# coezbek/Zonos

Hardware: AMD Instinct MI355X
Metric: DAC codes/sec (end-to-end generate + DAC decode), Zonos-v0.1-transformer batch=64/GPU (higher is better)
Workload: dtype bf16; 1 GPU; c3: B=64/GPU, Lc=400, prefix 10, 2580 new tokens (30 s), EOS disabled, CLI sampling (linear .65 conf .4 rep 2.5/8), DAC decode of all codes; model=Zonos-v0.1-transformer, global_batch=64, seq_len=2999, parallelism=dp1

## Files before the change

include/zonos_hip.h:

```cpp
#ifndef ZONOS_HIP_H
#define ZONOS_HIP_H
#include <stddef.h>
#include <stdint.h>

#ifdef __cplusplus
extern "C" {
#endif

int zk_version(void);
const char* zk_last_error(void);
int zk_device_sync(void);
long zk_abi_size(int which);

typedef struct zk_sampling_params {
    float temperature;
    float top_p;
    float min_p;
    float linear, conf, quad;
    int32_t top_k;
    int32_t rp_window;
    float cfg_scale;
    int32_t force_full_length;
} zk_sampling_params;

// ... 271 lines not shown
int zk_dac_rvq_decode(const int64_t* codes, int B, int ncb, int T, long code_bstride,
                      const float* tables, int ncode, int hidden, float* z, int Tz,
                      const int32_t* lens, void* stream);
int zk_dac_conv(const float* in, int B, int Cin, int Tin, const float* alpha,
                const float* w, const float* bias, int Cout, int ks, int dil, int pad,
                int Qn, int out_stride, int out_off, float* out, int Tout, const float* resid,
                int do_tanh, const int32_t* lens, int in_scale, int out_scale, void* stream);
int zk_dac_prep_convt(const float* w, int Cin, int Cout, int s, float* w_out, void* stream);

int zk_dac_prep_w16(const float* w, int Cout, int Cin, int ks, int s, int mode, uint16_t* w_hi,
                    uint16_t* w_lo, void* stream);
int zk_dac_conv16(const float* in, int B, int Cin, int Tin, const float* alpha, const uint16_t* w_hi,
                  const uint16_t* w_lo, const float* bias, int Cout, int ks, int dil, int pad,
                  int Qn, int out_stride, int out_off, float* out, int Tout, const float* resid,
                  int do_tanh, const int32_t* lens, int in_scale, int out_scale, int npass, void* stream);
int zk_dac_tail(const float* in, int B, int C, int T, const float* alpha, const float* w,
                const float* bias, float* out, const int32_t* lens, int scale, void* stream);

int zk_dac_rvq_decode_cl(const int64_t* codes, int B, int ncb, int T, long code_bstride,
                         const float* tables, int ncode, int hidden, int cpad, uint16_t* z,
                         const int32_t* lens, void* stream);
int zk_dac_conv_cl(const uint16_t* in, int B, int Cin, int Tin, const uint16_t* w, long w_phase_stride,
                   const float* bias, int Cout, int ks, int dil, int pad, int Qn, int nphase,
                   int out_stride, int out_off0, int Tout, const float* resid, float* x_out,
                   const float* alpha_next, void* s_out, int s_f32, const int32_t* lens, int in_scale,
                   int out_scale, void* stream);
int zk_dac_resunit_supported(int C);
int zk_dac_resunit_cl(const uint16_t* s_in, int B, int C, int T, const uint16_t* w7, const float* b7, int dil,
                      const float* a2, const uint16_t* w1, const float* b1, float* x, const float* alpha_next,
                      void* s_out, int s_f32, const int32_t* lens, int scale, void* stream);
#define ZK_DAC_PLAN_N 9
int zk_dac_conv_plan(int fused, int B, int Cin, int Cout, int ks, int dil, int Qn, int nphase, int resid,
                     int s_f32, int32_t* plan);
int zk_dac_tail_cl(const float* s, int B, int C, int T, const float* w, const float* bias,
                   float* out, const int32_t* lens, int scale, void* stream);

#define ZK_DAC_MAXB 6
#define ZK_DAC_MAXR 3
typedef struct zk_dac_resunit {
    int32_t dil;
    const float* a1;
    const uint16_t* w1;
    const float* b1;
    const float* a2;
    const uint16_t* w2;
    const float* b2;
} zk_dac_resunit;
typedef struct zk_dac_block {
    int32_t stride, cin, cout, nres;
    const float* alpha;
    const uint16_t* wt;
    const float* bt;
    zk_dac_resunit res[ZK_DAC_MAXR];
} zk_dac_block;
typedef struct zk_dac_desc {
    int32_t nblocks, ncb, codebook_size, hidden, cin0, c0;
    const float* tables;
    const uint16_t* conv1_w;
    const float* conv1_b;
    const float* final_alpha;
    const float* conv2_w;
    const float* conv2_b;
    zk_dac_block blocks[ZK_DAC_MAXB];
} zk_dac_desc;
size_t zk_dac_decode_workspace(const zk_dac_desc* d, int B, int T);
int zk_dac_decode(const zk_dac_desc* d, const int64_t* codes, int B, int T, const int32_t* lens, void* workspace,
// ... 107 lines not shown
```

zonos_amd/_lib.py:

```python
from __future__ import annotations

import ctypes as C
import os

import torch

_HERE = os.path.dirname(os.path.abspath(__file__))
LIB_PATH = os.environ.get("ZK_LIB_PATH") or os.path.join(_HERE, "lib", "libzonos_hip.so")

P = C.c_void_p
I = C.c_int
L = C.c_long
F = C.c_float
U64 = C.c_uint64
I64 = C.c_int64


class SamplingParams(C.Structure):
    _fields_ = [("temperature", F), ("top_p", F), ("min_p", F), ("linear", F), ("conf", F), ("quad", F),
                ("top_k", C.c_int32), ("rp_window", C.c_int32), ("cfg_scale", F),
                ("force_full_length", C.c_int32)]


class GenState(C.Structure):
# ... 167 lines not shown
}

_lib = None


class ZonosHipError(RuntimeError):
    pass


def load():
    global _lib
    if _lib is not None:
        return _lib
    if not os.path.exists(LIB_PATH):
        raise ZonosHipError(f"{LIB_PATH} not found: build it with `python -m zonos_amd.build` "
                            "(there is no CPU fallback)")
    lib = C.CDLL(LIB_PATH)
    for name, args in _SIGS.items():
        fn = getattr(lib, name)
        fn.argtypes = args
        fn.restype = C.c_int
    lib.zk_last_error.restype = C.c_char_p
    lib.zk_last_error.argtypes = []
    lib.zk_loudness_max_blocks.restype = C.c_int
    lib.zk_loudness_max_blocks.argtypes = [L, I]
    lib.zk_abi_size.restype = C.c_long
    lib.zk_abi_size.argtypes = [I]
    lib.zk_dac_decode_workspace.restype = C.c_size_t
    lib.zk_dac_decode_workspace.argtypes = [C.POINTER(DacDesc), I, I]
    lib.zk_stream_workspace.restype = C.c_size_t
    lib.zk_stream_workspace.argtypes = [C.POINTER(StreamDesc), I]
    lib.zk_dac_resunit_supported.restype = C.c_int
    lib.zk_dac_resunit_supported.argtypes = [I]
    lib.zk_gemm_warm_tiles.restype = C.c_int
    lib.zk_gemm_warm_tiles.argtypes = [I, I, I, I, I, I]
    lib.zk_torch_noise_policy.restype = C.c_int
    lib.zk_torch_noise_policy.argtypes = [L, I, I, C.POINTER(C.c_int), C.POINTER(C.c_long)]
    lib.zk_spk_conv_tiles.restype = C.c_int
    lib.zk_spk_conv_tiles.argtypes = [I, I]
    lib.zk_speaker_workspace_bytes.restype = C.c_size_t
    lib.zk_speaker_workspace_bytes.argtypes = [C.POINTER(SpkDesc), I, I]
    _lib = lib
    return lib


def exported_symbols() -> list[str]:
    return list(_SIGS) + ["zk_last_error", "zk_loudness_max_blocks", "zk_abi_size",
                          "zk_dac_decode_workspace", "zk_stream_workspace", "zk_dac_resunit_supported", "zk_gemm_warm_tiles",
                          "zk_torch_noise_policy", "zk_spk_conv_tiles", "zk_speaker_workspace_bytes"]


def call(name: str, *args):
    lib = load()
    if len(args) != len(_SIGS[name]):
        raise TypeError(f"{name}: {len(args)} arguments given, the C ABI takes {len(_SIGS[name])}")
    rc = getattr(lib, name)(*args)
    if rc != 0:
        raise ZonosHipError(f"{name} failed ({rc}): {lib.zk_last_error().decode()}")
    return rc


DAC_PLAN_FIELDS = ("shape", "fm", "tile", "dx", "nx", "lds", "nq", "tiles", "wg_per_cu")


def dac_conv_plan(B, Cin, Cout, ks, dil, Qn, nphase=1, resid=False, s_f32=False, fused=False) -> dict:
    plan = (C.c_int32 * len(DAC_PLAN_FIELDS))()
    call("zk_dac_conv_plan", int(fused), B, Cin, Cout, ks, dil, Qn, nphase, int(resid), int(s_f32), plan)
    return dict(zip(DAC_PLAN_FIELDS, plan))


def ptr(t) -> int | None:
    if t is None:
        return None
    return t.data_ptr()


def stream_ptr(device=None) -> int:
    return torch.cuda.current_stream(device).cuda_stream


def device_index(device) -> int:
    device = torch.device(device)
    return device.index if device.index is not None else torch.cuda.current_device()


def require_gpu(t: torch.Tensor, name: str = "tensor"):
    if not t.is_cuda:
        raise ZonosHipError(f"{name} must be a GPU tensor (the HIP engine has no CPU path)")
```

zonos_amd/csrc/dac_cl.hip:

```cpp
#include "common.h"
#include "../../include/zonos_hip.h"
#include <algorithm>
#include <stdlib.h>

namespace {

typedef __attribute__((ext_vector_type(8))) _Float16 f16x8;
typedef __attribute__((ext_vector_type(4))) float f32x4;

constexpr int MAXSPAN = 64;

__device__ __attribute__((aligned(256))) uint4 g_zero_page[16];

template <int CI>
struct Img {
    static constexpr int G = CI / 8;
    static constexpr int RB = CI * 2;
    static constexpr int RPB = 256 / RB;
    static constexpr int RPR = 4096 / RB;
    ZK_DEV static int swz(int row) { return (int)(((unsigned)row / RPB) % G); }
    ZK_DEV static int off(int row, int g) { return row * RB + ((g ^ swz(row)) << 4); }
};

ZK_DEV f16x8 as_h8(uint4 v) { return __builtin_bit_cast(f16x8, v); }
// ... 17 lines not shown

ZK_DEV void wait_vm(int n) {
#define ZK_W1(N_) case N_: asm volatile("s_waitcnt vmcnt(" #N_ ")" ::: "memory"); break;
#define ZK_W8(B_) ZK_W1(B_ + 0) ZK_W1(B_ + 1) ZK_W1(B_ + 2) ZK_W1(B_ + 3) ZK_W1(B_ + 4) ZK_W1(B_ + 5) ZK_W1(B_ + 6) ZK_W1(B_ + 7)
    switch (n < 0 ? 0 : (n > 63 ? 63 : n)) {
        ZK_W8(0) ZK_W8(8) ZK_W8(16) ZK_W8(24) ZK_W8(32) ZK_W8(40) ZK_W8(48) ZK_W8(56)
        default: asm volatile("s_waitcnt vmcnt(0)" ::: "memory"); break;
    }
#undef ZK_W8
#undef ZK_W1
}

#ifndef ZK_CL_DA
#define ZK_CL_DA 3
#endif
#ifdef ZK_CL_PROF
__device__ uint64_t g_clprof[64][3][64];
__device__ uint64_t g_clprof_end[64][2];
__device__ uint64_t g_clprof_rt[64][6];
__device__ uint64_t g_clwg[4096][2];
__device__ uint32_t g_clhw[4096][8];
#define ZK_CL_STAMP(role, st)                                                                          \
    do {                                                                                               \
        if (blockIdx.x < 64 && (st) < 64 && lane == 0) g_clprof[blockIdx.x][role][st] = __builtin_amdgcn_s_memtime(); \
    } while (0)
#else
#define ZK_CL_STAMP(role, st) do { } while (0)
#endif
constexpr int CL_DA = ZK_CL_DA;
#ifndef ZK_CL_NLD
#define ZK_CL_NLD 2
#endif
constexpr int CL_NLD = ZK_CL_NLD;

constexpr int RU_XPD = 4;
template <int NQ_, int DA_, int OCC_, int NWY_, int NLDK_, int NWM_, bool FUSE_, int FMF_ = 0>
struct ConvShape {
    static constexpr int NQ = NQ_, DA = DA_, OCC = OCC_, NWY = NWY_, NLDK = NLDK_, NWM = NWM_, FMF = FMF_;
    static constexpr bool FUSE = FUSE_;
    static constexpr int THREADS = 64 * (NWM * NWY + NLDK);
    static constexpr int QTT = 16 * NQ * NWY;
    static constexpr int co_t(int fm) { return 16 * fm * NWM; }
    static constexpr bool w1lds(int fm) { return FUSE && OCC == 1 && co_t(fm) * (co_t(fm) + 8) * 2 <= 24 * 1024; }
};
using ShapePair = ConvShape<4, CL_DA, 2, 2, CL_NLD, 2, false>;
using ShapeFat = ConvShape<8, CL_DA, 1, 4, 4, 2, false>;
using ShapeFused96 = ConvShape<4, CL_DA, 1, 8, 4, 1, true, 6>;
using ShapeFused192 = ConvShape<2, CL_DA, 1, 8, 4, 1, true, 12>;

struct ConvLds {
    int ws, nws, ept, w1;
    static constexpr int pieces(int win) { return (win + 15) >> 4; }
    static constexpr int xs(int nxp) { return nxp * 1024; }
    template <class P> constexpr P xring(P base) const { return base + nws * ws; }
    template <class P> constexpr P tables(P base, int nx, int xs_) const { return xring(base) + nx * xs_; }
    template <class P> constexpr P w1img(P base, int nx, int xs_) const { return tables(base, nx, xs_) + 2 * ept; }
    constexpr int bytes(int nx, int xs_) const { return w1img(0, nx, xs_) + w1; }
};
template <class S>
constexpr ConvLds conv_lds(int fm) {
    const int co_t = S::co_t(fm);
    return ConvLds{co_t * 64, S::DA + 2, (S::FUSE ? 6 : 3) * co_t * (int)sizeof(float),
                   S::w1lds(fm) ? co_t * (co_t + 8) * 2 : 0};
}

template <class S, int FM, bool SF32, bool RES>
__global__ __launch_bounds__(S::THREADS, (S::OCC * S::THREADS + 255) / 256) void k_conv_cl(
    const uint16_t* __restrict__ in, int Cin, int Tin, const uint16_t* __restrict__ w, long wphase,
    const float* __restrict__ bias, int Cout, int ks, int dil, int pad, int Qn, int nphase, int out_stride,
    int out_off0, int Tout, const float* resid, float* xout, const float* __restrict__ alpha,
    void* __restrict__ sout, int s_f32, const int32_t* __restrict__ lens, int in_scale, int out_scale, int nq,
    int nx_slots, int dx, int B, const uint16_t* __restrict__ w1x1, const float* __restrict__ b1x1,
    const float* __restrict__ alpha_out) {
    constexpr int NQ = S::NQ, DA = S::DA, NWY = S::NWY, NLDK = S::NLDK, NWM = S::NWM;
    constexpr bool FUSE = S::FUSE;
    constexpr ConvLds LDS = conv_lds<S>(FM);
// ... 2 lines not shown
    constexpr int CO_T = S::co_t(FM);
    constexpr int WS = LDS.ws;
    static_assert(WS == CO_T * I::RB, "weight slot = CO_T image rows");
    constexpr int NWP = CO_T / 16;
    constexpr int NCW = NWM * NWY;
    static_assert(!FUSE || (NWM == 1 && !RES), "fused residual unit: one channel wave, residual in the epilogue");
    constexpr int W1S = CO_T + 8;
    constexpr bool W1LDS = S::w1lds(FM);
    constexpr int QTT = S::QTT;
    extern __shared__ __attribute__((aligned(16))) char smem[];

    const int nco = (Cout / CO_T) * nphase;
    const int ntiles = B * nq * nco;
    const int kx = blockIdx.x >> 3, nper = gridDim.x >> 3;
    const int lo = (int)((long)(blockIdx.x & 7) * ntiles / 8), hi = (int)((long)((blockIdx.x & 7) + 1) * ntiles / 8);
    const int nt = hi - lo > kx ? (hi - lo - kx + nper - 1) / nper : 0;
    auto tile_of = [&](int i, int& b, int& phase, int& co0, int& q0) {
        const int L = lo + kx + i * nper;
        const int cot = L % nco;
        b = L / (nco * nq);
        q0 = ((L / nco) % nq) * QTT;
        phase = cot % nphase;
        co0 = (cot / nphase) * CO_T;
    };

    const int tid = threadIdx.x, lane = tid & 63, wv = __builtin_amdgcn_readfirstlane(tid >> 6);
    const int win = QTT + (ks - 1) * dil;
    const int nxp = ConvLds::pieces(win);
    const int XS = ConvLds::xs(nxp);
    constexpr int NWS = LDS.nws;
    char* const wring = smem;
    char* const xring = LDS.xring(smem);
    const int nchunk = Cin / CI, nstep = nchunk * ks;

#ifdef ZK_CL_PROF
    if (blockIdx.x < 4096 && lane == 0 && wv < 6) {
        g_clhw[blockIdx.x][wv] = __builtin_amdgcn_s_getreg((31 << 11) | 4);
        if (wv == 0) g_clhw[blockIdx.x][6] = __builtin_amdgcn_s_getreg((31 << 11) | 20);
    }
    if (wv == 0 && blockIdx.x < 4096 && lane == 0) g_clwg[blockIdx.x][0] = __builtin_amdgcn_s_memrealtime();
    if (wv == 0 && blockIdx.x < 64 && lane == 0) {
        g_clprof_rt[blockIdx.x][0] = __builtin_amdgcn_s_memrealtime();
        g_clprof_rt[blockIdx.x][4] = __builtin_amdgcn_s_memtime();
    }
#endif
    if (wv >= NCW) {
        const int lw = __builtin_amdgcn_readfirstlane(wv - NCW);
        const size_t wtap = (size_t)Cout * Cin;
        static_assert((16 / I::RPB) % I::G == 0, "piece-invariant swizzle needs 16-row pieces to span whole swizzle periods");
        const int prow = lane >> 2, pslot = lane & 3;
        const int g = pslot ^ I::swz(prow);
        const int loff = prow * Cin + g * 8;
        const long prs = 16L * Cin;
        const int nxl = (nxp - lw + NLDK - 1) / NLDK, nwl = (NWP - lw + NLDK - 1) / NLDK;
        int ix = 0, tx = 0, cx = 0, u0 = 0, len_in = Tin;
        bool xfast = false;
        const uint16_t* xsrc0 = in;
        auto set_xtile = [&](int i) {
            int b_, ph_, co_, q_;
            tile_of(i, b_, ph_, co_, q_);
            len_in = lens ? min(lens[b_] * in_scale, Tin) : Tin;
            u0 = q_ - pad;
            xsrc0 = in + (size_t)b_ * Tin * Cin + loff + (long)u0 * Cin;
            xfast = u0 >= 0 && u0 + nxp * 16 <= len_in;
        };
        int iw = 0, tw = 0, cw = 0;
        const uint16_t* wsrc0 = w;
        auto set_wtile = [&](int i) {
            int b_, ph_, co_, q_;
            tile_of(i, b_, ph_, co_, q_);
            wsrc0 = w + (size_t)ph_ * wphase + (size_t)co_ * Cin + loff;
        };
        if (nt > 0) {
            set_xtile(0);
            set_wtile(0);
        }
        int xslot = 0, wslot = 0;
        int hist[DA + 1] = {};
        const int total = nt * nstep;
        for (int j = -dx; j < total; ++j) {
            int nl = 0;
            if (ix < nt) {
                if (tx == 0) {
                    char* dst = xring + xslot * XS;
                    const uint16_t* src = xsrc0 + cx * CI;
                    if (xfast) {
                        for (int p = lw; p < nxp; p += NLDK)
                            __builtin_amdgcn_global_load_lds((const void*)(src + p * prs), (void*)(dst + p * 1024), 16,
                                                             0, 0);
                    } else {
                        for (int p = lw; p < nxp; p += NLDK) {
                            const int row = p * 16 + prow, u = u0 + row;
                            const void* sp = (row < win && u >= 0 && u < len_in) ? (const void*)(src + p * prs)
                                                                                 : (const void*)g_zero_page;
                            __builtin_amdgcn_global_load_lds(sp, (void*)(dst + p * 1024), 16, 0, 0);
                        }
                    }
                    nl += nxl;
                    if (++xslot == nx_slots) xslot = 0;
                }
                if (++tx == ks) {
                    tx = 0;
                    if (++cx == nchunk) {
                        cx = 0;
                        if (++ix < nt) set_xtile(ix);
                    }
                }
            }
            if (j + DA >= 0 && iw < nt) {
                char* dst = wring + wslot * WS;
                const uint16_t* src = wsrc0 + tw * wtap + cw * CI;
#pragma unroll
                for (int pp = 0; pp < (NWP + NLDK - 1) / NLDK; ++pp) {
                    const int p = pp * NLDK + lw;
                    if (p >= NWP) break;
                    __builtin_amdgcn_global_load_lds((const void*)(src + p * prs), (void*)(dst + p * 1024), 16, 0, 0);
                }
                nl += nwl;
                if (++wslot == NWS) wslot = 0;
                if (++tw == ks) {
                    tw = 0;
                    if (++cw == nchunk) {
                        cw = 0;
                        if (++iw < nt) set_wtile(iw);
                    }
                }
            }
#pragma unroll
            for (int k = 0; k < DA; ++k) hist[k] = hist[k + 1];
            hist[DA] = nl;
            if (j >= 0) {
                int pend = 0;
#pragma unroll
                for (int k = 1; k <= DA; ++k) pend += hist[k];
                if (lw == 0) ZK_CL_STAMP(0, j);
                wait_vm(pend);
                __builtin_amdgcn_s_barrier();
                if (lw == 0) ZK_CL_STAMP(1, j);
            }
        }
        return;
    }

    const int ln = lane & 15, lg = lane >> 4, wm = wv / NWY, wn = wv % NWY;
    int t = 0, xslot = 0, wslot = 0;
    constexpr int NE = FUSE ? 6 : 3;
    static_assert(LDS.ept == NE * CO_T * (int)sizeof(float), "epilogue table = NE rows of CO_T floats");
    uint16_t* const w1img = reinterpret_cast<uint16_t*>(LDS.w1img(smem, nx_slots, XS));
    if constexpr (W1LDS) {
        for (int i = tid; i < CO_T * CO_T / 8; i += 64 * NCW) {
            const int row = i / (CO_T / 8), c8 = i % (CO_T / 8);
            *reinterpret_cast<uint4*>(w1img + row * W1S + c8 * 8) =
                *reinterpret_cast<const uint4*>(w1x1 + (size_t)row * CO_T + c8 * 8);
        }
    }
    for (int it = 0; it < nt; ++it) {
        int b, phase, co0, q0;
        tile_of(it, b, phase, co0, q0);
        f32x4 acc[FM][NQ];
#pragma unroll
        for (int m = 0; m < FM; ++m)
#pragma unroll
            for (int n = 0; n < NQ; ++n) acc[m][n] = f32x4{0.f, 0.f, 0.f, 0.f};

        float* const ept = reinterpret_cast<float*>(LDS.tables(smem, nx_slots, XS)) + (it & 1) * NE * CO_T;
        for (int i = tid; i < CO_T; i += 64 * NCW) {
            const float a_ = (FUSE || sout) ? alpha[co0 + i] : 1.f;
            ept[i] = bias[co0 + i];
            ept[CO_T + i] = a_;
            ept[2 * CO_T + i] = __fdiv_rn(1.0f, __fadd_rn(a_, 1e-9f));
            if constexpr (FUSE) {
                const float an = alpha_out[i];
                ept[3 * CO_T + i] = b1x1[i];
                ept[4 * CO_T + i] = an;
                ept[5 * CO_T + i] = __fdiv_rn(1.0f, __fadd_rn(an, 1e-9f));
            }
        }
        asm volatile("s_waitcnt lgkmcnt(0)" ::: "memory");
        const int len_out = lens ? lens[b] * out_scale : Tout;

        float4 rv[RES ? FM : 1][NQ];
        if constexpr (RES) {
#pragma unroll
            for (int m = 0; m < FM; ++m)
#pragma unroll
                for (int n = 0; n < NQ; ++n) {
                    const int q = q0 + wn * 16 * NQ + n * 16 + ln;
                    const int tt = min(max(q * out_stride + out_off0 + phase, 0), Tout - 1);
                    rv[m][n] = *reinterpret_cast<const float4*>(
                        resid + ((size_t)b * Tout + tt) * Cout + co0 + wm * 16 * FM + m * 16 + lg * 4);
                }
        }

        for (int s = 0; s < nstep; ++s) {
            __builtin_amdgcn_s_barrier();
            asm volatile("" ::: "memory");
            if (wv == 0 && it == 0) ZK_CL_STAMP(2, s);
#ifdef ZK_CL_PROF
            if (it == 0 && s == 0 && wv == 0 && blockIdx.x < 64 && lane == 0)
                g_clprof_rt[blockIdx.x][1] = __builtin_amdgcn_s_memrealtime();
#endif
            const char* xb = xring + xslot * XS;
            const char* wb = wring + wslot * WS;
            if (++wslot == NWS) wslot = 0;
            uint4 a[FM], bq[NQ];
#pragma unroll
            for (int m = 0; m < FM; ++m)
                a[m] = *reinterpret_cast<const uint4*>(wb + I::off(wm * 16 * FM + m * 16 + ln, lg));
#pragma unroll
            for (int n = 0; n < NQ; ++n)
                bq[n] = *reinterpret_cast<const uint4*>(xb + I::off(wn * 16 * NQ + n * 16 + ln + t * dil, lg));
#pragma unroll
            for (int m = 0; m < FM; ++m)
#pragma unroll
                for (int n = 0; n < NQ; ++n)
                    acc[m][n] = __builtin_amdgcn_mfma_f32_16x16x32_f16(as_h8(a[m]), as_h8(bq[n]), acc[m][n], 0, 0, 0);
            if (++t == ks) {
                t = 0;
                if (++xslot == nx_slots) xslot = 0;
            }
        }

#ifdef ZK_CL_PROF
        if (it == 0 && wv == 0 && blockIdx.x < 64 && lane == 0) {
            float keep = 0.f;
#pragma unroll
            for (int m = 0; m < FM; ++m)
#pragma unroll
                for (int n = 0; n < NQ; ++n) keep += acc[m][n][0];
            g_clprof_end[blockIdx.x][0] = __builtin_amdgcn_s_memtime() + (keep == 1.2345f);
            g_clprof_rt[blockIdx.x][2] = __builtin_amdgcn_s_memrealtime();
        }
#endif
        const int out_off = out_off0 + phase;
        if constexpr (FUSE) {
            uint2 h[FM][NQ];
#pragma unroll
            for (int m = 0; m < FM; ++m) {
                const int cl = m * 16 + lg * 4;
                const float4 bb = *reinterpret_cast<const float4*>(ept + cl);
                const float4 aa = *reinterpret_cast<const float4*>(ept + CO_T + cl);
                const float4 rr = *reinterpret_cast<const float4*>(ept + 2 * CO_T + cl);
#pragma unroll
                for (int n = 0; n < NQ; ++n)
                    h[m][n] = pack_h4(snake_fast(__fadd_rn(acc[m][n][0], bb.x), aa.x, rr.x),
                                      snake_fast(__fadd_rn(acc[m][n][1], bb.y), aa.y, rr.y),
                                      snake_fast(__fadd_rn(acc[m][n][2], bb.z), aa.z, rr.z),
                                      snake_fast(__fadd_rn(acc[m][n][3], bb.w), aa.w, rr.w));
            }
            constexpr int XPD = RU_XPD < FM ? RU_XPD : FM;
            float4 xr[XPD][NQ];
            auto load_x = [&](int mo, int buf) {
#pragma unroll
                for (int n = 0; n < NQ; ++n) {
                    const int q = q0 + wn * 16 * NQ + n * 16 + ln;
                    const int tt = min(max(q * out_stride + out_off, 0), Tout - 1);
                    xr[buf][n] = *reinterpret_cast<const float4*>(resid + ((size_t)b * Tout + tt) * Cout + mo * 16 + lg * 4);
                }
            };
#pragma unroll
            for (int p = 0; p < XPD; ++p) load_x(p, p);
            const uint16_t* w1p = w1x1;
            asm volatile("" : "+s"(w1p));
            uint2 wf[2][W1LDS ? 1 : FM];
            auto load_w = [&](int mo, int buf) {
                if constexpr (!W1LDS) {
// ... 16 lines not shown
#pragma unroll
                    for (int n = 0; n < NQ; ++n)
                        z[n] = __builtin_amdgcn_mfma_f32_16x16x16f16(as_h4(wa), as_h4(h[m][n]), z[n], 0, 0, 0);
                }
                const int co = mo * 16 + lg * 4;
                const float4 bb = *reinterpret_cast<const float4*>(ept + 3 * CO_T + co);
                const float4 aa = *reinterpret_cast<const float4*>(ept + 4 * CO_T + co);
                const float4 rr = *reinterpret_cast<const float4*>(ept + 5 * CO_T + co);
#pragma unroll
                for (int n = 0; n < NQ; ++n) {
                    const int q = q0 + wn * 16 * NQ + n * 16 + ln;
                    const int tt = q * out_stride + out_off;
                    if (q >= Qn || tt < 0 || tt >= Tout) continue;
                    const size_t o = ((size_t)b * Tout + tt) * Cout + co;
                    float v0 = 0.f, v1 = 0.f, v2 = 0.f, v3 = 0.f;
                    if (tt < len_out) {
                        const float4 r = xr[mo % XPD][n];
                        v0 = __fadd_rn(r.x, __fadd_rn(z[n][0], bb.x));
                        v1 = __fadd_rn(r.y, __fadd_rn(z[n][1], bb.y));
                        v2 = __fadd_rn(r.z, __fadd_rn(z[n][2], bb.z));
                        v3 = __fadd_rn(r.w, __fadd_rn(z[n][3], bb.w));
                    }
                    *reinterpret_cast<float4*>(xout + o) = make_float4(v0, v1, v2, v3);
                    if (SF32)
                        reinterpret_cast<float4*>(sout)[o >> 2] =
                            make_float4(snake(v0, aa.x), snake(v1, aa.y), snake(v2, aa.z), snake(v3, aa.w));
                    else
                        *reinterpret_cast<uint2*>(reinterpret_cast<uint16_t*>(sout) + o) =
                            pack_h4(snake_fast(v0, aa.x, rr.x), snake_fast(v1, aa.y, rr.y),
                                    snake_fast(v2, aa.z, rr.z), snake_fast(v3, aa.w, rr.w));
                }
                if (mo + XPD < FM) load_x(mo + XPD, mo % XPD);
            }
            continue;
        }
#pragma unroll
        for (int m = 0; m < FM; ++m) {
            const int cl = wm * 16 * FM + m * 16 + lg * 4, co = co0 + cl;
            const float4 bb = *reinterpret_cast<const float4*>(ept + cl);
            const float4 aa = *reinterpret_cast<const float4*>(ept + CO_T + cl);
            const float4 rr = *reinterpret_cast<const float4*>(ept + 2 * CO_T + cl);
            const float r0 = rr.x, r1 = rr.y, r2 = rr.z, r3 = rr.w;
#pragma unroll
            for (int n = 0; n < NQ; ++n) {
                const int q = q0 + wn * 16 * NQ + n * 16 + ln;
                const int tt = q * out_stride + out_off;
                if (q >= Qn || tt < 0 || tt >= Tout) continue;
                const size_t o = ((size_t)b * Tout + tt) * Cout + co;
                float v0 = 0.f, v1 = 0.f, v2 = 0.f, v3 = 0.f;
                if (tt < len_out) {
                    v0 = __fadd_rn(acc[m][n][0], bb.x);
                    v1 = __fadd_rn(acc[m][n][1], bb.y);
                    v2 = __fadd_rn(acc[m][n][2], bb.z);
                    v3 = __fadd_rn(acc[m][n][3], bb.w);
                    if constexpr (RES) {
                        const float4 r = rv[m][n];
                        v0 = __fadd_rn(r.x, v0);
                        v1 = __fadd_rn(r.y, v1);
                        v2 = __fadd_rn(r.z, v2);
                        v3 = __fadd_rn(r.w, v3);
                    }
                }
                if (xout) *reinterpret_cast<float4*>(xout + o) = make_float4(v0, v1, v2, v3);
                if (!sout) continue;
                if (SF32)
                    reinterpret_cast<float4*>(sout)[o >> 2] =
                        make_float4(snake(v0, aa.x), snake(v1, aa.y), snake(v2, aa.z), snake(v3, aa.w));
                else
                    *reinterpret_cast<uint2*>(reinterpret_cast<uint16_t*>(sout) + o) =
                        pack_h4(snake_fast(v0, aa.x, r0), snake_fast(v1, aa.y, r1), snake_fast(v2, aa.z, r2),
                                snake_fast(v3, aa.w, r3));
            }
        }
#ifdef ZK_CL_PROF
        if (it == 0 && wv == 0 && blockIdx.x < 64 && lane == 0) {
            asm volatile("s_waitcnt vmcnt(0)" ::: "memory");
            g_clprof_rt[blockIdx.x][3] = __builtin_amdgcn_s_memrealtime();
            g_clprof_rt[blockIdx.x][5] = __builtin_amdgcn_s_memtime();
        }
#endif
    }
#ifdef ZK_CL_PROF
    if (wv == 0 && blockIdx.x < 4096 && lane == 0) {
        asm volatile("s_waitcnt vmcnt(0)" ::: "memory");
        g_clwg[blockIdx.x][1] = __builtin_amdgcn_s_memrealtime();
    }
#endif
}

__global__ __launch_bounds__(256) void k_rvq_cl(const int64_t* __restrict__ codes, int ncb, int T, long bstr,
                                                const float* __restrict__ tables, int ncode, int hidden, int cpad,
                                                uint16_t* __restrict__ z, const int32_t* __restrict__ lens) {
    const int t = blockIdx.x, b = blockIdx.y;
    const int len = lens ? lens[b] : T;
    for (int ch = threadIdx.x * 4; ch < cpad; ch += 1024) {
        float s[4] = {0.f, 0.f, 0.f, 0.f};
        if (t < len && ch < hidden) {
            for (int k = 0; k < ncb; ++k) {
                int64_t cd = codes[b * bstr + (size_t)k * T + t];
                cd = cd < 0 ? 0 : (cd >= ncode ? ncode - 1 : cd);
                const float4 e = *reinterpret_cast<const float4*>(tables + ((size_t)k * ncode + cd) * hidden + ch);
                if (k == 0) {
                    s[0] = e.x; s[1] = e.y; s[2] = e.z; s[3] = e.w;
                } else {
                    s[0] = __fadd_rn(s[0], e.x); s[1] = __fadd_rn(s[1], e.y);
                    s[2] = __fadd_rn(s[2], e.z); s[3] = __fadd_rn(s[3], e.w);
                }
            }
        }
        *reinterpret_cast<uint2*>(z + ((size_t)b * T + t) * cpad + ch) = pack_h4(s[0], s[1], s[2], s[3]);
    }
}

constexpr int TAIL_T = 128;
// ... 167 lines not shown
template <class F>
auto with_shape(int shape, F&& f) {
    return shape == SHAPE_FAT ? f(ShapeFat{}) : shape == SHAPE_FUSED96 ? f(ShapeFused96{})
         : shape == SHAPE_FUSED192 ? f(ShapeFused192{}) : f(ShapePair{});
}
struct ConvPlan { int shape, fm, qt, dx, nx, lds, nq, tiles, occ; };

int conv_plan(const char* name, bool fused, int B, int Cin, int Cout, int ks, int dil, int Qn, int nphase, bool resid,
              bool s_f32, ConvPlan& p) {
    if (fused) {
        ZK_REQUIRE(Cout == 96 || Cout == 192, "%s: C=%d (the fused unit is built for C = 96 and 192)", name, Cout);
        ZK_REQUIRE(dil >= 1 && 6 * dil <= MAXSPAN, "%s: dil=%d", name, dil);
        ks = 7, nphase = 1;
        p.shape = Cout == 96 ? SHAPE_FUSED96 : SHAPE_FUSED192, p.fm = Cout / 16;
    } else {
        ZK_REQUIRE(Cin > 0 && Cin % 32 == 0, "%s: Cin=%d must be a multiple of 32", name, Cin);
        ZK_REQUIRE(Cout > 0 && Cout % 32 == 0, "%s: Cout=%d must be a multiple of 32", name, Cout);
        ZK_REQUIRE(ks >= 1 && ks <= 7 && dil >= 1 && (ks - 1) * dil <= MAXSPAN, "%s: ks=%d dil=%d", name, ks, dil);
        ZK_REQUIRE(nphase >= 1, "%s: bad arguments", name);
        const int nco = Cout / 32;
        p.fm = nco % 4 == 0 ? 4 : (nco % 3 == 0 ? 3 : (nco % 2 == 0 ? 2 : 1));
        p.shape = (!resid && !s_f32 && nphase == 1 && p.fm <= 3) ? SHAPE_FAT : SHAPE_PAIR;
    }
    return with_shape(p.shape, [&](auto shape) -> int {
        using S = decltype(shape);
        const ConvLds lay = conv_lds<S>(p.fm);
        const int xs = ConvLds::xs(ConvLds::pieces(S::QTT + (ks - 1) * dil));
        const int cap = 160 * 1024 / S::OCC;
        for (p.dx = std::max(S::DA, ks);; --p.dx) {
            p.nx = 1 + (p.dx + ks) / ks, p.lds = lay.bytes(p.nx, xs);
            if (p.dx <= S::DA || p.lds <= cap) break;
        }
        ZK_REQUIRE(p.lds <= 160 * 1024, "%s: LDS %d too large (Cout %d ks %d dil %d)", name, p.lds, Cout, ks, dil);
        p.qt = S::QTT, p.occ = S::OCC;
        p.nq = Qn > 0 ? (Qn + S::QTT - 1) / S::QTT : 0;
        const long tiles = (long)B * p.nq * (Cout / S::co_t(p.fm)) * nphase;
        ZK_REQUIRE(tiles < (1L << 31), "%s: too many tiles", name);
        p.tiles = (int)tiles;
        return 0;
    });
}

template <class S>
constexpr bool conv_has(int fm, bool sf32, bool res) {
    return S::FUSE ? (fm == S::FMF && !res) : S::OCC == 1 ? (fm <= 3 && !sf32 && !res) : fm <= 4;
}

template <class K, class... A>
int conv_launch_kernel(K kern, int threads, const ConvPlan& p, const char* name, hipStream_t st, A... args) {
    const size_t lds = (size_t)p.lds;
    const void* fn = reinterpret_cast<const void*>(kern);
    if (lds > 65536) (void)hipFuncSetAttribute(fn, hipFuncAttributeMaxDynamicSharedMemorySize, (int)lds);
    int dev = 0, ncu = 0, occ = 0;
    ZK_HIP(hipGetDevice(&dev));
    ZK_HIP(hipDeviceGetAttribute(&ncu, hipDeviceAttributeMultiprocessorCount, dev));
    ZK_HIP(hipOccupancyMaxActiveBlocksPerMultiprocessor(&occ, fn, threads, lds));
    ZK_REQUIRE(occ >= 1, "%s: kernel does not fit a CU (LDS %zu)", name, lds);
    const long resident = (long)ncu * occ / 8 * 8;
    const long grid = std::min<long>(((long)p.tiles + 7) / 8 * 8, std::max<long>(resident, 8));
    hipLaunchKernelGGL(kern, dim3((unsigned)grid), dim3(threads), lds, st, args...);
    ZK_CHECK_LAUNCH(name);
    return 0;
}

template <class... A>
int conv_launch(const ConvPlan& p, bool sf32, bool res, const char* name, hipStream_t st, A... args) {
// ... 47 lines not shown
    hipLaunchKernelGGL(k_rvq_cl, dim3(T, B), dim3(256), 0, (hipStream_t)stream, codes, ncb, T, code_bstride, tables,
                       ncode, hidden, cpad, z, lens);
    ZK_CHECK_LAUNCH("zk_dac_rvq_decode_cl");
    return 0;
}

extern "C" int zk_dac_conv_cl(const uint16_t* in, int B, int Cin, int Tin, const uint16_t* w, long w_phase_stride,
                              const float* bias, int Cout, int ks, int dil, int pad, int Qn, int nphase,
                              int out_stride, int out_off0, int Tout, const float* resid, float* x_out,
                              const float* alpha_next, void* s_out, int s_f32, const int32_t* lens, int in_scale,
                              int out_scale, void* stream) {
    const char* const name = "zk_dac_conv_cl";
    ConvPlan p;
    ZK_TRY(conv_plan(name, false, B, Cin, Cout, ks, dil, Qn, nphase, resid != nullptr, s_f32 != 0, p));
    ZK_REQUIRE(bias != nullptr && (s_out == nullptr || alpha_next != nullptr) && (s_out != nullptr || x_out != nullptr),
               "zk_dac_conv_cl: bad arguments");
    if (B == 0 || Qn <= 0) return 0;
    return conv_launch(p, s_f32 != 0, resid != nullptr, name, (hipStream_t)stream, in, Cin, Tin, w, w_phase_stride, bias,
                       Cout, ks, dil, pad, Qn, nphase, out_stride, out_off0, Tout, resid, x_out, alpha_next, s_out, s_f32,
                       lens, in_scale, out_scale, p.nq, p.nx, p.dx, B, nullptr, nullptr, nullptr);
}

extern "C" int zk_dac_conv_plan(int fused, int B, int Cin, int Cout, int ks, int dil, int Qn, int nphase, int resid,
                                int s_f32, int32_t* plan) {
    ConvPlan p;
    ZK_REQUIRE(plan != nullptr, "zk_dac_conv_plan: null plan");
    if (conv_plan("zk_dac_conv_plan", fused != 0, B, Cin, Cout, ks, dil, Qn, nphase, resid != 0, s_f32 != 0, p) != 0)
        return -1;
    const int32_t v[ZK_DAC_PLAN_N] = {p.shape, p.fm, p.qt, p.dx, p.nx, p.lds, p.nq, p.tiles, p.occ};
    std::copy(v, v + ZK_DAC_PLAN_N, plan);
    return 0;
}

extern "C" int zk_dac_resunit_supported(int C) { return C == 96 ? 1 : 0; }

extern "C" int zk_dac_resunit_cl(const uint16_t* s_in, int B, int C, int T, const uint16_t* w7, const float* b7,
                                 int dil, const float* a2, const uint16_t* w1, const float* b1, float* x,
                                 const float* alpha_next, void* s_out, int s_f32, const int32_t* lens, int scale,
                                 void* stream) {
    const char* const name = "zk_dac_resunit_cl";
    ConvPlan p;
    ZK_TRY(conv_plan(name, true, B, C, C, 7, dil, T, 1, false, s_f32 != 0, p));
    ZK_REQUIRE(s_in != nullptr && w7 && b7 && a2 && w1 && b1 && x && alpha_next && s_out,
               "zk_dac_resunit_cl: null argument");
    ZK_REQUIRE(s_out != static_cast<const void*>(s_in),
               "zk_dac_resunit_cl: s_out must not alias s_in (neighbouring tiles read it as their halo)");
    if (B == 0 || T <= 0) return 0;
    return conv_launch(p, s_f32 != 0, false, name, (hipStream_t)stream, s_in, C, T, w7, 0L, b7, C, 7, dil, 3 * dil, T, 1,
                       1, 0, T, x, x, a2, s_out, (int)(s_f32 != 0), lens, scale, scale, p.nq, p.nx, p.dx, B, w1, b1,
                       alpha_next);
}

#ifdef ZK_CL_PROF
extern "C" int zk_cl_prof_read(void* dst, void* dst_end) {
    if (hipMemcpyFromSymbol(dst, HIP_SYMBOL(g_clprof), sizeof(g_clprof)) != hipSuccess) return -1;
    if (hipMemcpyFromSymbol(dst_end, HIP_SYMBOL(g_clprof_rt), sizeof(g_clprof_rt)) != hipSuccess) return -1;
    return 0;
}
extern "C" int zk_cl_prof_read_wg(void* dst) {
    return hipMemcpyFromSymbol(dst, HIP_SYMBOL(g_clwg), sizeof(g_clwg)) == hipSuccess ? 0 : -1;
}
extern "C" int zk_cl_prof_read_hw(void* dst) {
    return hipMemcpyFromSymbol(dst, HIP_SYMBOL(g_clhw), sizeof(g_clhw)) == hipSuccess ? 0 : -1;
}
#endif

// ... 15 lines not shown
```

Measured before the change: 159,400 codes/s.

## Prefetch next-step LDS operands during MFMA in DAC conv compute waves

Factors the loader and compute schedules of the DAC channels-last conv kernel into shared host/device schedule templates, and adds a host-callable schedule dump for testing. For the non-fused fat shape (no residual, no f32 output), compute waves now read the next step's weight and window fragments from LDS while the current step's MFMAs run, using a double-buffered A register set and sched_barriers. This is meant to hide LDS read latency behind MFMA work. The cost is extra VGPR pressure and an explicit waitcnt before each barrier.

```diff
diff --git a/include/zonos_hip.h b/include/zonos_hip.h
--- a/include/zonos_hip.h
+++ b/include/zonos_hip.h
@@ -327,6 +327,11 @@
 #define ZK_DAC_PLAN_N 9
 int zk_dac_conv_plan(int fused, int B, int Cin, int Cout, int ks, int dil, int Qn, int nphase, int resid,
                      int s_f32, int32_t* plan);
+#define ZK_DAC_SCHED_EV 4
+enum { ZK_DAC_SCHED_LOADER = 0, ZK_DAC_SCHED_COMPUTE = 1 };
+enum { ZK_DAC_EV_BARRIER = 0, ZK_DAC_EV_WINDOW = 1, ZK_DAC_EV_WEIGHTS = 2, ZK_DAC_EV_MFMA = 3, ZK_DAC_EV_TILE_END = 4 };
+int zk_dac_conv_schedule(int role, int ahead, int tiles, int nchunk, int ks, int dx, int da, int nx, int nws,
+                         int32_t* events, int cap);
 int zk_dac_tail_cl(const float* s, int B, int C, int T, const float* w, const float* bias,
                    float* out, const int32_t* lens, int scale, void* stream);
 
diff --git a/zonos_amd/_lib.py b/zonos_amd/_lib.py
--- a/zonos_amd/_lib.py
+++ b/zonos_amd/_lib.py
@@ -223,6 +223,8 @@
     lib.zk_stream_workspace.argtypes = [C.POINTER(StreamDesc), I]
     lib.zk_dac_resunit_supported.restype = C.c_int
     lib.zk_dac_resunit_supported.argtypes = [I]
+    lib.zk_dac_conv_schedule.restype = C.c_int
+    lib.zk_dac_conv_schedule.argtypes = [I] * 9 + [P, I]
     lib.zk_gemm_warm_tiles.restype = C.c_int
     lib.zk_gemm_warm_tiles.argtypes = [I, I, I, I, I, I]
     lib.zk_torch_noise_policy.restype = C.c_int
@@ -237,7 +239,7 @@
 
 def exported_symbols() -> list[str]:
     return list(_SIGS) + ["zk_last_error", "zk_loudness_max_blocks", "zk_abi_size",
-                          "zk_dac_decode_workspace", "zk_stream_workspace", "zk_dac_resunit_supported", "zk_gemm_warm_tiles",
+                          "zk_dac_decode_workspace", "zk_stream_workspace", "zk_dac_resunit_supported", "zk_dac_conv_schedule", "zk_gemm_warm_tiles",
                           "zk_torch_noise_policy", "zk_spk_conv_tiles", "zk_speaker_workspace_bytes"]
 
 
@@ -260,6 +262,21 @@
     return dict(zip(DAC_PLAN_FIELDS, plan))
 
 
+DAC_EV_BARRIER, DAC_EV_WINDOW, DAC_EV_WEIGHTS, DAC_EV_MFMA, DAC_EV_TILE_END = range(5)
+
+
+def dac_conv_schedule(role, ahead, tiles, nchunk, ks, dx, da, nx, nws) -> list[tuple] | None:
+    lib = load()
+    args = (int(role), int(ahead), tiles, nchunk, ks, dx, da, nx, nws)
+    n = lib.zk_dac_conv_schedule(*args, None, 0)
+    if n < 0:
+        return None
+    ev = (C.c_int32 * (4 * n))()
+    if lib.zk_dac_conv_schedule(*args, ev, n) != n:
+        raise ZonosHipError("zk_dac_conv_schedule: event count changed between calls")
+    return [tuple(ev[4 * i:4 * i + 4]) for i in range(n)]
+
+
 def ptr(t) -> int | None:
     if t is None:
         return None
diff --git a/zonos_amd/csrc/dac_cl.hip b/zonos_amd/csrc/dac_cl.hip
--- a/zonos_amd/csrc/dac_cl.hip
+++ b/zonos_amd/csrc/dac_cl.hip
@@ -73,6 +73,100 @@
 #define ZK_CL_NLD 2
 #endif
 constexpr int CL_NLD = ZK_CL_NLD;
+constexpr bool CL_AHEAD_FAT = true, CL_AHEAD_PAIR = false;
+
+#define ZK_HD __host__ __device__ __forceinline__
+struct ConvSched {
+    int nt, nchunk, ks;
+    int dx, da;
+    int nx, nws;
+    ZK_HD int nstep() const { return nchunk * ks; }
+    ZK_HD int total() const { return nt * nstep(); }
+    ZK_HD bool valid() const {
+        return nt >= 0 && nchunk >= 1 && ks >= 1 && da >= 1 && dx >= da && nws >= da + 2 && (nx - 1) * ks >= dx + 1;
+    }
+};
+template <int V> using SchedInt = std::integral_constant<int, V>;
+
+template <class TX, class TW, class FX, class FW, class FE, class FP>
+ZK_HD void conv_sched_loader(const ConvSched& c, TX&& x_tile, TW&& w_tile, FX&& issue_x, FW&& issue_w, FE&& end_issue,
+                             FP&& publish) {
+    const int total = c.total();
+    int ix = 0, cx = 0, tx = 0, xslot = 0;
+    int iw = 0, cw = 0, tw = 0, wslot = 0;
+    if (c.nt > 0) {
+        x_tile(0);
+        w_tile(0);
+    }
+    for (int j = -c.dx; j < total; ++j) {
+        if (ix < c.nt) {
+            if (tx == 0) {
+                issue_x(j, ix, cx, xslot);
+                if (++xslot == c.nx) xslot = 0;
+            }
+            if (++tx == c.ks) {
+                tx = 0;
+                if (++cx == c.nchunk) {
+                    cx = 0;
+                    if (++ix < c.nt) x_tile(ix);
+                }
+            }
+        }
+        if (j + c.da >= 0 && iw < c.nt) {
+            issue_w(j, iw, cw, tw, wslot);
+            if (++wslot == c.nws) wslot = 0;
+            if (++tw == c.ks) {
+                tw = 0;
+                if (++cw == c.nchunk) {
+                    cw = 0;
+                    if (++iw < c.nt) w_tile(iw);
+                }
+            }
+        }
+        end_issue(j);
+        if (j >= 0) publish(j, c.da);
+    }
+}
+
+template <bool AHEAD, class TB, class SY, class RD, class ST, class RO, class TE>
+ZK_HD void conv_sched_compute(const ConvSched& c, TB&& tile_begin, SY&& sync, RD&& read, ST&& step, RO&& rotate,
+                              TE&& tile_end) {
+    using No = SchedInt<0>;
+    using Yes = SchedInt<1>;
+    const int nstep = c.nstep();
+    int g = 0, t = 0, xslot = 0, wslot = 0;
+    auto advance = [&] {
+        ++g;
+        if (++wslot == c.nws) wslot = 0;
+        if (++t == c.ks) {
+            t = 0;
+            if (++xslot == c.nx) xslot = 0;
+        }
+    };
+    for (int it = 0; it < c.nt; ++it) {
+        tile_begin(it);
+        if constexpr (!AHEAD) {
+            for (int s = 0; s < nstep; ++s) {
+                sync(g);
+                read(g, t, xslot, wslot);
+                advance();
+                step(No{}, g - 1, 0, 0, 0);
+            }
+        } else {
+            sync(g);
+            read(g, t, xslot, wslot);
+            advance();
+            for (int s = 1; s < nstep; ++s) {
+                sync(g);
+                step(Yes{}, g - 1, t, xslot, wslot);
+                advance();
+                rotate();
+            }
+            step(No{}, g - 1, 0, 0, 0);
+        }
+        tile_end(it);
+    }
+}
 
 constexpr int RU_XPD = 4;
 template <int NQ_, int DA_, int OCC_, int NWY_, int NLDK_, int NWM_, bool FUSE_, int FMF_ = 0>
@@ -83,6 +177,8 @@
     static constexpr int QTT = 16 * NQ * NWY;
     static constexpr int co_t(int fm) { return 16 * fm * NWM; }
     static constexpr bool w1lds(int fm) { return FUSE && OCC == 1 && co_t(fm) * (co_t(fm) + 8) * 2 <= 24 * 1024; }
+    static constexpr bool AHEAD = !FUSE && (OCC == 1 ? CL_AHEAD_FAT : CL_AHEAD_PAIR);
+    static constexpr int na2(int fm) { return fm - 1; }
 };
 using ShapePair = ConvShape<4, CL_DA, 2, 2, CL_NLD, 2, false>;
 using ShapeFat = ConvShape<8, CL_DA, 1, 4, 4, 2, false>;
@@ -151,6 +247,7 @@
     char* const wring = smem;
     char* const xring = LDS.xring(smem);
     const int nchunk = Cin / CI, nstep = nchunk * ks;
+    const ConvSched sched{nt, nchunk, ks, dx, DA, nx_slots, NWS};
 
 #ifdef ZK_CL_PROF
     if (blockIdx.x < 4096 && lane == 0 && wv < 6) {
@@ -172,7 +269,7 @@
         const int loff = prow * Cin + g * 8;
         const long prs = 16L * Cin;
         const int nxl = (nxp - lw + NLDK - 1) / NLDK, nwl = (NWP - lw + NLDK - 1) / NLDK;
-        int ix = 0, tx = 0, cx = 0, u0 = 0, len_in = Tin;
+        int u0 = 0, len_in = Tin;
         bool xfast = false;
         const uint16_t* xsrc0 = in;
         auto set_xtile = [&](int i) {
@@ -183,50 +280,33 @@
             xsrc0 = in + (size_t)b_ * Tin * Cin + loff + (long)u0 * Cin;
             xfast = u0 >= 0 && u0 + nxp * 16 <= len_in;
         };
-        int iw = 0, tw = 0, cw = 0;
         const uint16_t* wsrc0 = w;
         auto set_wtile = [&](int i) {
             int b_, ph_, co_, q_;
             tile_of(i, b_, ph_, co_, q_);
             wsrc0 = w + (size_t)ph_ * wphase + (size_t)co_ * Cin + loff;
         };
-        if (nt > 0) {
-            set_xtile(0);
-            set_wtile(0);
-        }
-        int xslot = 0, wslot = 0;
         int hist[DA + 1] = {};
-        const int total = nt * nstep;
-        for (int j = -dx; j < total; ++j) {
-            int nl = 0;
-            if (ix < nt) {
-                if (tx == 0) {
-                    char* dst = xring + xslot * XS;
-                    const uint16_t* src = xsrc0 + cx * CI;
-                    if (xfast) {
-                        for (int p = lw; p < nxp; p += NLDK)
-                            __builtin_amdgcn_global_load_lds((const void*)(src + p * prs), (void*)(dst + p * 1024), 16,
-                                                             0, 0);
-                    } else {
-                        for (int p = lw; p < nxp; p += NLDK) {
-                            const int row = p * 16 + prow, u = u0 + row;
-                            const void* sp = (row < win && u >= 0 && u < len_in) ? (const void*)(src + p * prs)
-                                                                                 : (const void*)g_zero_page;
-                            __builtin_amdgcn_global_load_lds(sp, (void*)(dst + p * 1024), 16, 0, 0);
-                        }
+        int nl = 0;
+        conv_sched_loader(
+            sched, set_xtile, set_wtile,
+            [&](int, int, int cx, int xslot) {
+                char* dst = xring + xslot * XS;
+                const uint16_t* src = xsrc0 + cx * CI;
+                if (xfast) {
+                    for (int p = lw; p < nxp; p += NLDK)
+                        __builtin_amdgcn_global_load_lds((const void*)(src + p * prs), (void*)(dst + p * 1024), 16, 0, 0);
+                } else {
+                    for (int p = lw; p < nxp; p += NLDK) {
+                        const int row = p * 16 + prow, u = u0 + row;
+                        const void* sp = (row < win && u >= 0 && u < len_in) ? (const void*)(src + p * prs)
+                                                                             : (const void*)g_zero_page;
+                        __builtin_amdgcn_global_load_lds(sp, (void*)(dst + p * 1024), 16, 0, 0);
                     }
-                    nl += nxl;
-                    if (++xslot == nx_slots) xslot = 0;
-                }
-                if (++tx == ks) {
-                    tx = 0;
-                    if (++cx == nchunk) {
-                        cx = 0;
-                        if (++ix < nt) set_xtile(ix);
-                    }
-                }
-            }
-            if (j + DA >= 0 && iw < nt) {
+                }
+                nl += nxl;
+            },
+            [&](int, int, int cw, int tw, int wslot) {
                 char* dst = wring + wslot * WS;
                 const uint16_t* src = wsrc0 + tw * wtap + cw * CI;
 #pragma unroll
@@ -236,19 +316,14 @@
                     __builtin_amdgcn_global_load_lds((const void*)(src + p * prs), (void*)(dst + p * 1024), 16, 0, 0);
                 }
                 nl += nwl;
-                if (++wslot == NWS) wslot = 0;
-                if (++tw == ks) {
-                    tw = 0;
-                    if (++cw == nchunk) {
-                        cw = 0;
-                        if (++iw < nt) set_wtile(iw);
-                    }
-                }
-            }
-#pragma unroll
-            for (int k = 0; k < DA; ++k) hist[k] = hist[k + 1];
-            hist[DA] = nl;
-            if (j >= 0) {
+            },
+            [&](int) {
+#pragma unroll
+                for (int k = 0; k < DA; ++k) hist[k] = hist[k + 1];
+                hist[DA] = nl;
+                nl = 0;
+            },
+            [&](int j, int) {
                 int pend = 0;
 #pragma unroll
                 for (int k = 1; k <= DA; ++k) pend += hist[k];
@@ -256,13 +331,13 @@
                 wait_vm(pend);
                 __builtin_amdgcn_s_barrier();
                 if (lw == 0) ZK_CL_STAMP(1, j);
-            }
-        }
+            });
         return;
     }
 
     const int ln = lane & 15, lg = lane >> 4, wm = wv / NWY, wn = wv % NWY;
-    int t = 0, xslot = 0, wslot = 0;
+    constexpr bool AHEAD = S::AHEAD && !RES && !SF32;
+    constexpr int NA2 = AHEAD ? S::na2(FM) : 0;
     constexpr int NE = FUSE ? 6 : 3;
     static_assert(LDS.ept == NE * CO_T * (int)sizeof(float), "epilogue table = NE rows of CO_T floats");
     uint16_t* const w1img = reinterpret_cast<uint16_t*>(LDS.w1img(smem, nx_slots, XS));
@@ -273,16 +348,19 @@
                 *reinterpret_cast<const uint4*>(w1x1 + (size_t)row * CO_T + c8 * 8);
         }
     }
-    for (int it = 0; it < nt; ++it) {
-        int b, phase, co0, q0;
+    int b = 0, phase = 0, co0 = 0, q0 = 0, len_out = 0;
+    f32x4 acc[FM][NQ];
+    float* ept = nullptr;
+    float4 rv[RES ? FM : 1][NQ];
+    uint4 a[NA2 ? 2 : 1][FM], bq[1][NQ];
+    auto tile_begin = [&](int it) __attribute__((always_inline)) {
         tile_of(it, b, phase, co0, q0);
-        f32x4 acc[FM][NQ];
 #pragma unroll
         for (int m = 0; m < FM; ++m)
 #pragma unroll
             for (int n = 0; n < NQ; ++n) acc[m][n] = f32x4{0.f, 0.f, 0.f, 0.f};
 
-        float* const ept = reinterpret_cast<float*>(LDS.tables(smem, nx_slots, XS)) + (it & 1) * NE * CO_T;
+        ept = reinterpret_cast<float*>(LDS.tables(smem, nx_slots, XS)) + (it & 1) * NE * CO_T;
         for (int i = tid; i < CO_T; i += 64 * NCW) {
             const float a_ = (FUSE || sout) ? alpha[co0 + i] : 1.f;
             ept[i] = bias[co0 + i];
@@ -296,9 +374,8 @@
             }
         }
         asm volatile("s_waitcnt lgkmcnt(0)" ::: "memory");
-        const int len_out = lens ? lens[b] * out_scale : Tout;
-
-        float4 rv[RES ? FM : 1][NQ];
+        len_out = lens ? lens[b] * out_scale : Tout;
+
         if constexpr (RES) {
 #pragma unroll
             for (int m = 0; m < FM; ++m)
@@ -311,35 +388,72 @@
                 }
         }
 
-        for (int s = 0; s < nstep; ++s) {
-            __builtin_amdgcn_s_barrier();
-            asm volatile("" ::: "memory");
-            if (wv == 0 && it == 0) ZK_CL_STAMP(2, s);
+    };
+
+    auto sync = [&](int g) __attribute__((always_inline)) {
+        if constexpr (AHEAD) __builtin_amdgcn_s_waitcnt(0xc07f);
+        __builtin_amdgcn_s_barrier();
+        asm volatile("" ::: "memory");
+        if (wv == 0 && g < nstep) ZK_CL_STAMP(2, g);
 #ifdef ZK_CL_PROF
-            if (it == 0 && s == 0 && wv == 0 && blockIdx.x < 64 && lane == 0)
-                g_clprof_rt[blockIdx.x][1] = __builtin_amdgcn_s_memrealtime();
+        if (g == 0 && wv == 0 && blockIdx.x < 64 && lane == 0)
+            g_clprof_rt[blockIdx.x][1] = __builtin_amdgcn_s_memrealtime();
 #endif
-            const char* xb = xring + xslot * XS;
-            const char* wb = wring + wslot * WS;
-            if (++wslot == NWS) wslot = 0;
-            uint4 a[FM], bq[NQ];
+    };
+    auto read_a = [&](int set, int m, int wslot) __attribute__((always_inline)) {
+        a[set][m] = *reinterpret_cast<const uint4*>(wring + wslot * WS + I::off(wm * 16 * FM + m * 16 + ln, lg));
+    };
+    auto read_b = [&](int set, int n, int t, int xslot) __attribute__((always_inline)) {
+        bq[set][n] = *reinterpret_cast<const uint4*>(xring + xslot * XS + I::off(wn * 16 * NQ + n * 16 + ln + t * dil, lg));
+    };
+    auto read = [&](int, int t, int xslot, int wslot) __attribute__((always_inline)) {
+#pragma unroll
+        for (int m = 0; m < FM; ++m) read_a(0, m, wslot);
+#pragma unroll
+        for (int n = 0; n < NQ; ++n) read_b(0, n, t, xslot);
+    };
+    auto step = [&](auto next, int, int t, int xslot, int wslot) __attribute__((always_inline)) {
+        if constexpr (!AHEAD) {
 #pragma unroll
             for (int m = 0; m < FM; ++m)
-                a[m] = *reinterpret_cast<const uint4*>(wb + I::off(wm * 16 * FM + m * 16 + ln, lg));
-#pragma unroll
-            for (int n = 0; n < NQ; ++n)
-                bq[n] = *reinterpret_cast<const uint4*>(xb + I::off(wn * 16 * NQ + n * 16 + ln + t * dil, lg));
-#pragma unroll
-            for (int m = 0; m < FM; ++m)
 #pragma unroll
                 for (int n = 0; n < NQ; ++n)
-                    acc[m][n] = __builtin_amdgcn_mfma_f32_16x16x32_f16(as_h8(a[m]), as_h8(bq[n]), acc[m][n], 0, 0, 0);
-            if (++t == ks) {
-                t = 0;
-                if (++xslot == nx_slots) xslot = 0;
-            }
-        }
-
+                    acc[m][n] = __builtin_amdgcn_mfma_f32_16x16x32_f16(as_h8(a[0][m]), as_h8(bq[0][n]), acc[m][n], 0, 0, 0);
+        } else {
+            const char* const wb = wring + wslot * WS + I::off(wm * 16 * FM + ln, lg);
+            const char* const xb = xring + xslot * XS + I::off(wn * 16 * NQ + ln + t * dil, lg);
+            if constexpr (next() != 0) {
+#pragma unroll
+                for (int m = 0; m < NA2; ++m) a[1][m] = *reinterpret_cast<const uint4*>(wb + m * 16 * I::RB);
+            }
+            __builtin_amdgcn_sched_barrier(0);
+#pragma unroll
+            for (int n = 0; n < NQ; ++n) {
+#pragma unroll
+                for (int m = 0; m < FM; ++m) {
+                    acc[m][n] = __builtin_amdgcn_mfma_f32_16x16x32_f16(as_h8(a[0][m]), as_h8(bq[0][n]), acc[m][n], 0, 0, 0);
+                    if (next() != 0 && m >= NA2 && n == NQ - 1) {
+                        __builtin_amdgcn_sched_barrier(0);
+                        a[0][m] = *reinterpret_cast<const uint4*>(wb + m * 16 * I::RB);
+                        __builtin_amdgcn_sched_barrier(0);
+                    }
+                }
+                if constexpr (next() != 0) {
+                    __builtin_amdgcn_sched_barrier(0);
+                    bq[0][n] = *reinterpret_cast<const uint4*>(xb + n * 16 * I::RB);
+                    __builtin_amdgcn_sched_barrier(0);
+                }
+            }
+        }
+    };
+    auto rotate = [&]() __attribute__((always_inline)) {
+        if constexpr (AHEAD) {
+#pragma unroll
+            for (int m = 0; m < NA2; ++m) a[0][m] = a[1][m];
+        }
+    };
+
+    auto tile_end = [&](int it) __attribute__((always_inline)) {
 #ifdef ZK_CL_PROF
         if (it == 0 && wv == 0 && blockIdx.x < 64 && lane == 0) {
             float keep = 0.f;
@@ -351,6 +465,7 @@
             g_clprof_rt[blockIdx.x][2] = __builtin_amdgcn_s_memrealtime();
         }
 #endif
+        if constexpr (RES) asm volatile("" : "+s"(q0), "+s"(b), "+s"(co0));
         const int out_off = out_off0 + phase;
         if constexpr (FUSE) {
             uint2 h[FM][NQ];
@@ -433,7 +548,7 @@
                 }
                 if (mo + XPD < FM) load_x(mo + XPD, mo % XPD);
             }
-            continue;
+            return;
         }
 #pragma unroll
         for (int m = 0; m < FM; ++m) {
@@ -480,7 +595,8 @@
             g_clprof_rt[blockIdx.x][5] = __builtin_amdgcn_s_memtime();
         }
 #endif
-    }
+    };
+    conv_sched_compute<AHEAD>(sched, tile_begin, sync, read, step, rotate, tile_end);
 #ifdef ZK_CL_PROF
     if (wv == 0 && blockIdx.x < 4096 && lane == 0) {
         asm volatile("s_waitcnt vmcnt(0)" ::: "memory");
@@ -714,6 +830,8 @@
             if (p.dx <= S::DA || p.lds <= cap) break;
         }
         ZK_REQUIRE(p.lds <= 160 * 1024, "%s: LDS %d too large (Cout %d ks %d dil %d)", name, p.lds, Cout, ks, dil);
+        ZK_REQUIRE((ConvSched{0, 1, ks, p.dx, S::DA, p.nx, lay.nws}).valid(), "%s: rings too small for the schedule (ks %d dx %d nx %d)",
+                   name, ks, p.dx, p.nx);
         p.qt = S::QTT, p.occ = S::OCC;
         p.nq = Qn > 0 ? (Qn + S::QTT - 1) / S::QTT : 0;
         const long tiles = (long)B * p.nq * (Cout / S::co_t(p.fm)) * nphase;
@@ -827,6 +945,46 @@
     return 0;
 }
 
+extern "C" int zk_dac_conv_schedule(int role, int ahead, int tiles, int nchunk, int ks, int dx, int da, int nx,
+                                    int nws, int32_t* events, int cap) {
+    const ConvSched c{tiles, nchunk, ks, dx, da, nx, nws};
+    ZK_REQUIRE(role == ZK_DAC_SCHED_LOADER || role == ZK_DAC_SCHED_COMPUTE, "zk_dac_conv_schedule: role %d", role);
+    ZK_REQUIRE(c.valid(), "zk_dac_conv_schedule: not a schedule the kernel runs (tiles %d chunks %d ks %d dx %d da %d nx %d nws %d)",
+               tiles, nchunk, ks, dx, da, nx, nws);
+    ZK_REQUIRE(cap >= 0 && (cap == 0 || events != nullptr), "zk_dac_conv_schedule: bad buffer");
+    long n = 0;
+    auto put = [&](int kind, int step, int slot, int aux) {
+        if (n < cap) {
+            const int32_t v[ZK_DAC_SCHED_EV] = {kind, step, slot, aux};
+            std::copy(v, v + ZK_DAC_SCHED_EV, events + n * ZK_DAC_SCHED_EV);
+        }
+        ++n;
+    };
+    const int nstep = c.nstep();
+    if (role == ZK_DAC_SCHED_LOADER) {
+        conv_sched_loader(
+            c, [](int) {}, [](int) {},
+            [&](int j, int tile, int chunk, int slot) { put(ZK_DAC_EV_WINDOW, tile * nstep + chunk * ks, slot, j); },
+            [&](int j, int tile, int chunk, int tap, int slot) { put(ZK_DAC_EV_WEIGHTS, tile * nstep + chunk * ks + tap, slot, j); },
+            [](int) {}, [&](int j, int inflight) { put(ZK_DAC_EV_BARRIER, j, 0, j - inflight); });
+    } else {
+        auto sync = [&](int g) { put(ZK_DAC_EV_BARRIER, g, 0, 0); };
+        auto read = [&](int g, int t, int xslot, int wslot) {
+            put(ZK_DAC_EV_WEIGHTS, g, wslot, 0);
+            put(ZK_DAC_EV_WINDOW, g - t, xslot, t);
+        };
+        auto step = [&](auto next, int g, int t, int xslot, int wslot) {
+            if (next() != 0) read(g + 1, t, xslot, wslot);
+            put(ZK_DAC_EV_MFMA, g, 0, 0);
+        };
+        auto tile_end = [&](int it) { put(ZK_DAC_EV_TILE_END, (it + 1) * nstep - 1, 0, it); };
+        if (ahead) conv_sched_compute<true>(c, [](int) {}, sync, read, step, [] {}, tile_end);
+        else conv_sched_compute<false>(c, [](int) {}, sync, read, step, [] {}, tile_end);
+    }
+    ZK_REQUIRE(n < (1L << 31), "zk_dac_conv_schedule: too many events");
+    return (int)n;
+}
+
 extern "C" int zk_dac_resunit_supported(int C) { return C == 96 ? 1 : 0; }
 
 extern "C" int zk_dac_resunit_cl(const uint16_t* s_in, int B, int C, int T, const uint16_t* w7, const float* b7,
```

Result: no change. 158,800 codes/s (-0.4%).
